# saminiir/level-ip

Measured on AMD Instinct MI355X. Metric: device-resident checksum GB/s over packet batch; % of HBM-read roofline, higher is better.
Workload: dtype u16

## Files before the change

### level-ip_amd/csrc/push_kernels.hip

```cpp
#include <hip/hip_runtime.h>

#include <stdint.h>

#include "seg_frame_dev.h"

namespace lvlip {

constexpr uint32_t PUSH_WAVES = 4;

__global__ __launch_bounds__(256) void k_push_count(lvlip_snd_flow* s, const lvlip_push_flow* w, uint32_t nflows,
                                                    lvlip_frame_desc* fd, uint8_t* sacked, lvlip_push_result* res) {
    const uint32_t lane = threadIdx.x & 63u;
    const uint64_t k64 = (uint64_t)blockIdx.x * PUSH_WAVES + (threadIdx.x >> 6);
    if (k64 >= nflows) return;
    const uint32_t k = (uint32_t)k64;
    const uint32_t una = s[k].snd_una, nxt = s[k].snd_nxt, seg0 = s[k].seg0, nseg = s[k].nseg;
    const lvlip_push_flow* t = w + k;
    const uint32_t q0 = t->q0, cap = t->cap;

    const uint32_t moved = seg0 != q0 ? nseg : 0u;
    if (seg0 > q0 && nseg <= cap) {
        for (uint64_t c0 = 0; c0 < nseg; c0 += 64u) {
            const uint64_t i = c0 + lane;
            uint4 d = make_uint4(0u, 0u, 0u, 0u);
            uint8_t b = 0;
            if (i < nseg) {
                d = load_global(reinterpret_cast<uint64_t>(fd + (seg0 + (uint32_t)i)));
                if (sacked) b = sacked[seg0 + (uint32_t)i];
            }
            __builtin_amdgcn_wave_barrier();
            if (i < nseg) {
                store_global(reinterpret_cast<uint64_t>(fd + (q0 + (uint32_t)i)), u32x4{d.x, d.y, d.z, d.w});
                if (sacked) sacked[q0 + (uint32_t)i] = b;
            }
        }
    }

    if (lane == 0u) {
        const uint32_t unsent = t->unsent, mss = t->mss, wnd = t->wnd;
        const uint32_t span = nxt - una;
        const uint32_t need = mss ? (uint32_t)(((uint64_t)unsent + mss - 1u) / mss) : 0u;
        uint32_t m = nseg < cap && (seg0 >= q0 || nseg == 0u) ? cap - nseg : 0u;
        m = min(m, min(t->push, need));
        const bool open = span <= wnd;
        const uint32_t room = open ? wnd - span : 0u;
        const uint32_t fit = open && unsent <= room ? need : (mss ? room / mss : 0u);
        m = min(m, fit);
        const uint64_t by = (uint64_t)m * mss;
        const uint32_t bytes = by < unsent ? (uint32_t)by : unsent;
        store_global(reinterpret_cast<uint64_t>(res + k), u32x4{m, bytes, q0 + nseg, moved});
        s[k].seg0 = q0;
    }
}

__global__ __launch_bounds__(256) void k_push(const lvlip_lro_flow* f, const lvlip_lro_result* lro,
                                              const lvlip_snd_flow* s, const lvlip_push_flow* w, uint32_t nflows,
                                              uint32_t nslots, const uint8_t* payload, uint8_t* base,
                                              lvlip_frame_desc* fd, uint8_t* sacked, lvlip_frame_desc* fd_out,
                                              const lvlip_push_result* res) {
    const uint32_t tl = threadIdx.x & (TSO_ROW - 1u);
    const uint64_t g64 = (uint64_t)blockIdx.x * TSO_SEGS + (threadIdx.x / TSO_ROW);
    const bool inside = g64 < nslots;
    const uint32_t g = inside ? (uint32_t)g64 : 0u;

    const uint32_t k = slot_owner<&lvlip_push_flow::slot0>(w, nflows, g);
    const lvlip_push_flow* t = w + k;
    const uint4 r = load_global(reinterpret_cast<uint64_t>(res + k));
    const uint32_t i = g - t->slot0;
    const bool live = inside && g >= t->slot0 && i < t->push && i < r.x;
    const uint32_t mss = t->mss, unsent = t->unsent;
    const uint64_t done = (uint64_t)i * mss;
    const uint32_t dlen = live ? (unsent - done < mss ? (uint32_t)(unsent - done) : mss) : 0u;
    const bool last = done + dlen == unsent;

    uint64_t slot = (uint64_t)t->slot_nxt + i;
    if (slot >= t->cap) slot -= t->cap;
    const uint64_t off = live ? t->ring_off + slot * t->stride : 0ull;
    const uint64_t F = reinterpret_cast<uint64_t>(base) + off;
    const uint64_t S = reinterpret_cast<uint64_t>(payload) + t->pay_off + done;
    uint32_t h[14];
    tso_frame(tl, live, h, F, S, dlen, last, [=](uint32_t(&hd)[14]) {
        const uint32_t* hw = reinterpret_cast<const uint32_t*>(t->hdr);
#pragma unroll
        for (int j = 0; j < 14; ++j) hd[j] = hw[j];
        hdr_put_ack(hd, __builtin_bswap32(f[k].rcv_nxt + (lro ? lro[k].delivered : 0u)));
        hd[12] = (hd[12] & 0xffff0000u) | bswap16u(s[k].win);
        return s[k].snd_nxt + (uint32_t)done;
    });

    if (inside && tl == 0u) {
        const u32x4 d = live ? u32x4{(uint32_t)off, (uint32_t)(off >> 32), (uint32_t)TSO_HDR + dlen, 0u}
                             : u32x4{0u, 0u, 0u, 0u};
        store_global(reinterpret_cast<uint64_t>(fd_out + g), d);
        if (live) {
            store_global(reinterpret_cast<uint64_t>(fd + (r.z + i)), d);
            if (sacked) sacked[r.z + i] = 0;
        }
    }
}

__global__ __launch_bounds__(256) void k_push_step(lvlip_snd_flow* s, lvlip_push_flow* w, uint32_t nflows,
                                                   const lvlip_push_result* res) {
    const uint32_t k = blockIdx.x * 256u + threadIdx.x;
    if (k >= nflows) return;
    uint2* sw = reinterpret_cast<uint2*>(s + k);
    uint2* ww = reinterpret_cast<uint2*>(w + k);
    const uint4 r = load_global(reinterpret_cast<uint64_t>(res + k));
    uint2 a = sw[0], q = sw[1], p = ww[0], u = ww[2], n = ww[4];
    const uint32_t cap = ww[3].x;
    a.y += r.y;
    q.y += r.x;
    const uint64_t pay = (((uint64_t)p.y << 32) | p.x) + r.y;
    p.x = (uint32_t)pay, p.y = (uint32_t)(pay >> 32);
    u.x -= r.y;
    const uint64_t nx = (uint64_t)n.x + r.x;
    n.x = (uint32_t)(nx >= cap ? nx - cap : nx);
    sw[0] = a, sw[1] = q;
    ww[0] = p, ww[2] = u, ww[4] = n;
}

}

extern "C" {

int lvlip_push_dev(const lvlip_lro_flow* f, const lvlip_lro_result* lro, lvlip_snd_flow* s, lvlip_push_flow* w,
                   uint32_t nflows, uint32_t nslots, const void* payload, void* base, lvlip_frame_desc* fd,
                   uint8_t* sacked, lvlip_frame_desc* fd_out, lvlip_push_result* res, void* stream) {
    if (nflows > LVLIP_LRO_MAX_FLOWS || nslots > LVLIP_MAX_BATCH) return LVLIP_EINVAL;
    if (nslots && (!payload || !base || !fd_out || nflows == 0)) return LVLIP_EINVAL;
    if (nflows == 0) return LVLIP_OK;
    if (!f || !s || !w || !fd || !res) return LVLIP_EINVAL;
    if (((uintptr_t)f & 7u) || ((uintptr_t)s & 7u) || ((uintptr_t)w & 7u) || ((uintptr_t)lro & 15u) ||
        ((uintptr_t)fd & 15u) || ((uintptr_t)fd_out & 15u) || ((uintptr_t)res & 15u))
        return LVLIP_EINVAL;
    hipStream_t st = (hipStream_t)stream;
    const uint32_t fgrid = (nflows + lvlip::PUSH_WAVES - 1u) / lvlip::PUSH_WAVES;
    hipLaunchKernelGGL(lvlip::k_push_count, dim3(fgrid), dim3(256), 0, st, s, w, nflows, fd, sacked, res);
    int rc = lvlip_launched("k_push_count");
    if (rc != LVLIP_OK) return rc;
    if (nslots) {
        const uint32_t grid = (uint32_t)(((uint64_t)nslots + lvlip::TSO_SEGS - 1u) / lvlip::TSO_SEGS);
        hipLaunchKernelGGL(lvlip::k_push, dim3(grid), dim3(256), 0, st, f, lro, s, w, nflows, nslots,
                           (const uint8_t*)payload, (uint8_t*)base, fd, sacked, fd_out, res);
        rc = lvlip_launched("k_push");
        if (rc != LVLIP_OK) return rc;
    }
    hipLaunchKernelGGL(lvlip::k_push_step, dim3((nflows + 255u) / 256u), dim3(256), 0, st, s, w, nflows, res);
    return lvlip_launched("k_push_step");
}

}
```

### level-ip_amd/csrc/seg_frame_dev.h

```cpp
#pragma once

#include <hip/hip_runtime.h>

#include <stdint.h>

#include "csum_dev.h"
#include "row_copy.h"
#include "tcp_hdr_dev.h"

namespace lvlip {

constexpr uint32_t TSO_ROW = 16;
constexpr uint32_t TSO_SEGS = 256 / TSO_ROW;
constexpr int TSO_U = 4;
constexpr int TSO_HDR = TCP_FRAME_HDR;

template <class PATCH>
__device__ __forceinline__ void tso_frame(uint32_t tl, bool live, uint32_t (&h)[14], uint64_t F, uint64_t S,
                                          uint32_t dlen, bool last, PATCH&& patch) {
    const int f = (int)(F & 15ull);
    const uint64_t D = F - (uint64_t)f;
    const int L = TSO_HDR + (int)dlen;
    const uint32_t nch = live ? (uint32_t)(f + L + 15) >> 4 : 0u;
    const uint32_t hk = (uint32_t)(f + TSO_HDR + 15) >> 4;
    const uint32_t sel = (F & 1ull) ? 0x02030001u : 0x03020100u;

    uint32_t acc = 0;
    uint4 keep = make_uint4(0u, 0u, 0u, 0u);
    for (uint32_t k0 = 0; k0 < nch; k0 += TSO_ROW * TSO_U) {
        uint4 v[TSO_U];
        row_gather<TSO_U, true>(S, f + TSO_HDR, dlen, nch, k0, tl, v);
#pragma unroll
        for (int u = 0; u < TSO_U; ++u) {
            const uint32_t k = k0 + (uint32_t)u * TSO_ROW + tl;
            acc = chunk_acc(v[u], sel, acc);
            if (k < nch) {
                if (k >= hk) store_chunk(D + 16ull * k, v[u], 0, min(16, f + L - (int)(16u * k)));
                else keep = v[u];
            }
        }
    }
    const uint32_t W = row_sum_dpp(acc);

    const uint32_t seq = patch(h);
    h[13] &= 0xffffu;
    h[4] = (h[4] & 0xffff0000u) | bswap16u(40u + dlen);
    h[6] &= 0xffff0000u;
    const uint32_t ipw = (h[3] >> 16) + halves(h[4]) + halves(h[5]) + halves(h[6]) + halves(h[7]) +
                         (h[8] & 0xffffu);
    h[6] |= (uint32_t)finish(0u, ipw);
    const uint32_t nseq = __builtin_bswap32(seq);
    h[9] = (h[9] & 0xffffu) | (nseq << 16);
    h[10] = (h[10] & 0xffff0000u) | (nseq >> 16);
    if (!last) h[11] &= ~(0x09u << 24);
    h[12] &= 0xffffu;
    const uint32_t thw = hdr_tcp_words(h);
    h[12] |= (uint32_t)finish(hdr_tcp_seed(h, 20u + dlen), thw + W) << 16;

    if (tl < hk && tl < nch) {
        const uint4 blk[4] = {make_uint4(h[0], h[1], h[2], h[3]), make_uint4(h[4], h[5], h[6], h[7]),
                              make_uint4(h[8], h[9], h[10], h[11]), make_uint4(h[12], h[13], 0u, 0u)};
        const uint4 hv = hdr_chunk(tl, f, blk);
        const uint4 v = make_uint4(keep.x | hv.x, keep.y | hv.y, keep.z | hv.z, keep.w | hv.w);
        store_chunk(D + 16ull * tl, v, tl == 0u ? f : 0, min(16, f + L - (int)(16u * tl)));
    }
}

}
```

### level-ip_amd/csrc/seg_kernels.hip

```cpp
#include <hip/hip_runtime.h>

#include <stdint.h>

#include "seg_frame_dev.h"

namespace lvlip {

__global__ __launch_bounds__(256) void k_tso(const uint8_t* payload, const lvlip_tso_send* s, uint32_t n,
                                             uint32_t nseg, uint8_t* out, lvlip_frame_desc* fd) {
    const uint32_t tl = threadIdx.x & (TSO_ROW - 1u);
    const uint64_t g64 = (uint64_t)blockIdx.x * TSO_SEGS + (threadIdx.x / TSO_ROW);
    bool live = g64 < nseg;
    const uint32_t g = live ? (uint32_t)g64 : 0u;

    const lvlip_tso_send* t = s + slot_owner<&lvlip_tso_send::seg0>(s, n, g);
    const uint32_t mss = t->mss, len = t->len;
    const uint32_t i = g - t->seg0;
    const uint64_t done = (uint64_t)i * mss;
    live = live && g >= t->seg0 && done < len;
    const uint32_t dlen = live ? (len - done < mss ? (uint32_t)(len - done) : mss) : 0u;
    const bool last = done + dlen == len;

    uint32_t h[14];
    {
        const uint32_t* hw = reinterpret_cast<const uint32_t*>(t->hdr);
#pragma unroll
        for (int k = 0; k < 14; ++k) h[k] = hw[k];
    }

    const uint64_t off = t->out_off + (uint64_t)i * t->stride;
    const uint64_t F = reinterpret_cast<uint64_t>(out) + off;
    const uint64_t S = reinterpret_cast<uint64_t>(payload) + t->payload_off + done;
    const uint32_t seq0 = __builtin_bswap32((h[9] >> 16) | (h[10] << 16));
    tso_frame(tl, live, h, F, S, dlen, last, [=](uint32_t(&)[14]) { return seq0 + (uint32_t)done; });
    if (fd && live && tl == 0u)
        store_global(reinterpret_cast<uint64_t>(fd + g), u32x4{(uint32_t)off, (uint32_t)(off >> 32), (uint32_t)TSO_HDR + dlen, 0u});
}

}

extern "C" {

int lvlip_tso_dev(const void* payload, const lvlip_tso_send* s, uint32_t n, uint32_t nseg, void* out,
                  lvlip_frame_desc* fd, void* stream) {
    if (n == 0) return LVLIP_OK;
    if (!payload || !s || !out || nseg == 0 || nseg > LVLIP_MAX_BATCH) return LVLIP_EINVAL;
    const uint32_t grid = (uint32_t)(((uint64_t)nseg + lvlip::TSO_SEGS - 1u) / lvlip::TSO_SEGS);
    hipLaunchKernelGGL(lvlip::k_tso, dim3(grid), dim3(256), 0, (hipStream_t)stream, (const uint8_t*)payload, s,
                       n, nseg, (uint8_t*)out, fd);
    return lvlip_launch_status(hipGetLastError(), "k_tso");
}

}
```

Before: 6883.

## Software-pipeline TSO payload loads and make k_tso a persistent grid-stride kernel

Measured after the change: 6882 (median of 2 runs). No clear change (-0.0%).

```diff
diff --git a/level-ip_amd/csrc/push_kernels.hip b/level-ip_amd/csrc/push_kernels.hip
--- a/level-ip_amd/csrc/push_kernels.hip
+++ b/level-ip_amd/csrc/push_kernels.hip
@@ -79,7 +79,7 @@
     const uint64_t F = reinterpret_cast<uint64_t>(base) + off;
     const uint64_t S = reinterpret_cast<uint64_t>(payload) + t->pay_off + done;
     uint32_t h[14];
-    tso_frame(tl, live, h, F, S, dlen, last, [=](uint32_t(&hd)[14]) {
+    tso_frame(tl, live, h, F, S, dlen, last, reinterpret_cast<uint64_t>(w), [=](uint32_t(&hd)[14]) {
         const uint32_t* hw = reinterpret_cast<const uint32_t*>(t->hdr);
 #pragma unroll
         for (int j = 0; j < 14; ++j) hd[j] = hw[j];
diff --git a/level-ip_amd/csrc/seg_frame_dev.h b/level-ip_amd/csrc/seg_frame_dev.h
--- a/level-ip_amd/csrc/seg_frame_dev.h
+++ b/level-ip_amd/csrc/seg_frame_dev.h
@@ -12,37 +12,79 @@
 
 constexpr uint32_t TSO_ROW = 16;
 constexpr uint32_t TSO_SEGS = 256 / TSO_ROW;
-constexpr int TSO_U = 4;
+constexpr int TSO_U = 3;
+constexpr uint32_t TSO_ROUND = TSO_ROW * TSO_U;
 constexpr int TSO_HDR = TCP_FRAME_HDR;
 
-template <class PATCH>
-__device__ __forceinline__ void tso_frame(uint32_t tl, bool live, uint32_t (&h)[14], uint64_t F, uint64_t S,
-                                          uint32_t dlen, bool last, PATCH&& patch) {
-    const int f = (int)(F & 15ull);
-    const uint64_t D = F - (uint64_t)f;
-    const int L = TSO_HDR + (int)dlen;
-    const uint32_t nch = live ? (uint32_t)(f + L + 15) >> 4 : 0u;
-    const uint32_t hk = (uint32_t)(f + TSO_HDR + 15) >> 4;
-    const uint32_t sel = (F & 1ull) ? 0x02030001u : 0x03020100u;
+struct tso_seg {
+    uint64_t D, A0;
+    uint32_t dlen;
+    uint32_t nch;
+    uint32_t sh;
+    uint32_t j0, j1;
+    int f;
+};
 
-    uint32_t acc = 0;
-    uint4 keep = make_uint4(0u, 0u, 0u, 0u);
-    for (uint32_t k0 = 0; k0 < nch; k0 += TSO_ROW * TSO_U) {
-        uint4 v[TSO_U];
-        row_gather<TSO_U, true>(S, f + TSO_HDR, dlen, nch, k0, tl, v);
+__device__ __forceinline__ tso_seg tso_seg_at(bool live, uint64_t F, uint64_t S, uint32_t dlen, uint64_t safe) {
+    tso_seg q;
+    q.f = (int)(F & 15ull);
+    q.D = F - (uint64_t)q.f;
+    const uint64_t A = S - (uint64_t)(q.f + TSO_HDR);
+    const bool has = live && dlen != 0u;
+    q.A0 = has ? A & ~15ull : safe;
+    q.sh = (uint32_t)(A & 15ull);
+    q.dlen = live ? dlen : 0u;
+    q.nch = live ? (uint32_t)(q.f + TSO_HDR + (int)dlen + 15) >> 4 : 0u;
+    q.j0 = has ? (uint32_t)(((S & ~15ull) - q.A0) >> 4) : 0u;
+    q.j1 = has ? (uint32_t)((((S + dlen - 1u) & ~15ull) - q.A0) >> 4) : 0u;
+    return q;
+}
+
+__device__ __forceinline__ void tso_issue(const tso_seg& q, uint32_t k0, uint32_t tl, uint4 (&x)[TSO_U + 1]) {
 #pragma unroll
-        for (int u = 0; u < TSO_U; ++u) {
-            const uint32_t k = k0 + (uint32_t)u * TSO_ROW + tl;
-            acc = chunk_acc(v[u], sel, acc);
-            if (k < nch) {
-                if (k >= hk) store_chunk(D + 16ull * k, v[u], 0, min(16, f + L - (int)(16u * k)));
-                else keep = v[u];
-            }
+    for (int u = 0; u < TSO_U; ++u) {
+        const uint32_t j = k0 + (uint32_t)u * TSO_ROW + tl;
+        x[u] = load_nt_global(q.A0 + 16ull * min(max(j, q.j0), q.j1));
+    }
+    x[TSO_U] = load_nt_global(q.A0 + 16ull * min(max(k0 + TSO_ROUND, q.j0), q.j1));
+}
+
+__device__ __forceinline__ uint32_t row_next(uint32_t v) {
+    return (uint32_t)__builtin_amdgcn_update_dpp(0, (int)v, 0x12F, 0xF, 0xF, false);
+}
+
+__device__ __forceinline__ void tso_consume(const tso_seg& q, uint32_t k0, uint32_t tl, const uint4 (&x)[TSO_U + 1],
+                                            uint32_t& acc, uint4& keep) {
+    const int lead = q.f + TSO_HDR;
+    const int L = TSO_HDR + (int)q.dlen;
+    const uint32_t hk = (uint32_t)(lead + 15) >> 4;
+    const uint32_t sel = (q.f & 1) ? 0x02030001u : 0x03020100u;
+#pragma unroll
+    for (int u = 0; u < TSO_U; ++u) {
+        const uint32_t k = k0 + (uint32_t)u * TSO_ROW + tl;
+        const int rel = (int)(16u * k) - lead;
+        const int jlo = min(max(-rel, 0), 16);
+        const int jhi = min(max((int)q.dlen - rel, 0), 16);
+        const uint4 own = x[u], nxt = x[u + 1];
+        const uint4 hi = make_uint4(row_next(tl == 0u ? nxt.x : own.x), row_next(tl == 0u ? nxt.y : own.y),
+                                    row_next(tl == 0u ? nxt.z : own.z), row_next(tl == 0u ? nxt.w : own.w));
+        const uint4 v = mask_chunk(funnel16(own, hi, q.sh), jlo, jhi);
+        acc = chunk_acc(v, sel, acc);
+        if (k < q.nch) {
+            if (k >= hk) store_chunk(q.D + 16ull * k, v, 0, min(16, q.f + L - (int)(16u * k)));
+            else keep = v;
         }
     }
+}
+
+__device__ __forceinline__ void tso_finish(const tso_seg& q, uint32_t tl, uint32_t (&h)[14], uint32_t acc,
+                                           const uint4 keep, bool last, uint32_t seq) {
+    const uint32_t dlen = q.dlen;
+    const int f = q.f;
+    const int L = TSO_HDR + (int)dlen;
+    const uint32_t hk = (uint32_t)(f + TSO_HDR + 15) >> 4;
     const uint32_t W = row_sum_dpp(acc);
 
-    const uint32_t seq = patch(h);
     h[13] &= 0xffffu;
     h[4] = (h[4] & 0xffff0000u) | bswap16u(40u + dlen);
     h[6] &= 0xffff0000u;
@@ -57,13 +99,33 @@
     const uint32_t thw = hdr_tcp_words(h);
     h[12] |= (uint32_t)finish(hdr_tcp_seed(h, 20u + dlen), thw + W) << 16;
 
-    if (tl < hk && tl < nch) {
+    if (tl < hk && tl < q.nch) {
         const uint4 blk[4] = {make_uint4(h[0], h[1], h[2], h[3]), make_uint4(h[4], h[5], h[6], h[7]),
                               make_uint4(h[8], h[9], h[10], h[11]), make_uint4(h[12], h[13], 0u, 0u)};
         const uint4 hv = hdr_chunk(tl, f, blk);
         const uint4 v = make_uint4(keep.x | hv.x, keep.y | hv.y, keep.z | hv.z, keep.w | hv.w);
-        store_chunk(D + 16ull * tl, v, tl == 0u ? f : 0, min(16, f + L - (int)(16u * tl)));
+        store_chunk(q.D + 16ull * tl, v, tl == 0u ? f : 0, min(16, f + L - (int)(16u * tl)));
     }
 }
 
+template <class PATCH>
+__device__ __forceinline__ void tso_frame(uint32_t tl, bool live, uint32_t (&h)[14], uint64_t F, uint64_t S,
+                                          uint32_t dlen, bool last, uint64_t safe, PATCH&& patch) {
+    const tso_seg q = tso_seg_at(live, F, S, dlen, safe);
+    uint32_t acc = 0;
+    uint4 keep = make_uint4(0u, 0u, 0u, 0u);
+    uint4 xa[TSO_U + 1], xb[TSO_U + 1];
+    tso_issue(q, 0u, tl, xa);
+    for (uint32_t k0 = 0;; k0 += 2u * TSO_ROUND) {
+        tso_issue(q, k0 + TSO_ROUND, tl, xb);
+        tso_consume(q, k0, tl, xa, acc, keep);
+        if (k0 + TSO_ROUND >= q.nch) break;
+        tso_issue(q, k0 + 2u * TSO_ROUND, tl, xa);
+        tso_consume(q, k0 + TSO_ROUND, tl, xb, acc, keep);
+        if (k0 + 2u * TSO_ROUND >= q.nch) break;
+    }
+    const uint32_t seq = patch(h);
+    tso_finish(q, tl, h, acc, keep, last, seq);
 }
+
+}
diff --git a/level-ip_amd/csrc/seg_kernels.hip b/level-ip_amd/csrc/seg_kernels.hip
--- a/level-ip_amd/csrc/seg_kernels.hip
+++ b/level-ip_amd/csrc/seg_kernels.hip
@@ -6,35 +6,102 @@
 
 namespace lvlip {
 
+constexpr int TSO_WAVES_PER_CU = 8;
+
+struct tso_cache {
+    uint32_t idx;
+    uint32_t seg0, len, mss, stride;
+    uint64_t out_off, pay_off;
+    uint32_t h[14];
+};
+
+struct tso_job {
+    tso_seg q;
+    uint64_t off;
+    uint32_t g;
+    uint32_t seq;
+    bool last;
+};
+
+__device__ __forceinline__ tso_job tso_resolve(uint64_t g64, uint32_t nseg, const lvlip_tso_send* s, uint32_t n,
+                                               tso_cache& c, const uint8_t* payload, uint8_t* out) {
+    bool live = g64 < nseg;
+    const uint32_t g = live ? (uint32_t)g64 : 0u;
+    if (live) {
+        const bool hit = c.idx < n && g >= c.seg0 && (uint64_t)(g - c.seg0) * c.mss < c.len;
+        if (!hit) {
+            c.idx = slot_owner<&lvlip_tso_send::seg0>(s, n, g);
+            const lvlip_tso_send* t = s + c.idx;
+            c.seg0 = t->seg0, c.len = t->len, c.mss = t->mss, c.stride = t->stride;
+            c.out_off = t->out_off, c.pay_off = t->payload_off;
+            const uint32_t* hw = reinterpret_cast<const uint32_t*>(t->hdr);
+#pragma unroll
+            for (int k = 0; k < 14; ++k) c.h[k] = hw[k];
+        }
+    }
+    const uint32_t i = g - c.seg0;
+    const uint64_t done = (uint64_t)i * c.mss;
+    live = live && g >= c.seg0 && done < c.len;
+    const uint32_t dlen = live ? (c.len - done < c.mss ? (uint32_t)(c.len - done) : c.mss) : 0u;
+    tso_job j;
+    j.g = g;
+    j.last = done + dlen == c.len;
+    j.off = c.out_off + (uint64_t)i * c.stride;
+    j.seq = __builtin_bswap32((c.h[9] >> 16) | (c.h[10] << 16)) + (uint32_t)done;
+    j.q = tso_seg_at(live, reinterpret_cast<uint64_t>(out) + j.off,
+                     reinterpret_cast<uint64_t>(payload) + c.pay_off + done, dlen, reinterpret_cast<uint64_t>(s));
+    return j;
+}
+
+__device__ __forceinline__ void tso_step(uint32_t tl, const uint4 (&xc)[TSO_U + 1], uint4 (&xi)[TSO_U + 1],
+                                         tso_job& cur, uint32_t& k0, uint64_t& g, uint64_t R, uint32_t (&hc)[14],
+                                         uint32_t& acc, uint4& keep, tso_cache& c, const uint8_t* payload,
+                                         const lvlip_tso_send* s, uint32_t n, uint32_t nseg, uint8_t* out,
+                                         lvlip_frame_desc* fd) {
+    const bool more = k0 + TSO_ROUND < cur.q.nch;
+    tso_job nx = cur;
+    uint32_t nk0 = k0 + TSO_ROUND;
+    if (!more) {
+        g += R;
+        nx = tso_resolve(g, nseg, s, n, c, payload, out);
+        nk0 = 0u;
+    }
+    tso_issue(nx.q, nk0, tl, xi);
+    tso_consume(cur.q, k0, tl, xc, acc, keep);
+    if (!more) {
+        tso_finish(cur.q, tl, hc, acc, keep, cur.last, cur.seq);
+        if (fd && tl == 0u)
+            store_global(reinterpret_cast<uint64_t>(fd + cur.g),
+                         u32x4{(uint32_t)cur.off, (uint32_t)(cur.off >> 32), (uint32_t)TSO_HDR + cur.q.dlen, 0u});
+        acc = 0u;
+#pragma unroll
+        for (int k = 0; k < 14; ++k) hc[k] = c.h[k];
+    }
+    cur = nx;
+    k0 = nk0;
+}
+
 __global__ __launch_bounds__(256) void k_tso(const uint8_t* payload, const lvlip_tso_send* s, uint32_t n,
                                              uint32_t nseg, uint8_t* out, lvlip_frame_desc* fd) {
     const uint32_t tl = threadIdx.x & (TSO_ROW - 1u);
-    const uint64_t g64 = (uint64_t)blockIdx.x * TSO_SEGS + (threadIdx.x / TSO_ROW);
-    bool live = g64 < nseg;
-    const uint32_t g = live ? (uint32_t)g64 : 0u;
+    const uint64_t R = (uint64_t)gridDim.x * TSO_SEGS;
+    uint64_t g = (uint64_t)blockIdx.x * TSO_SEGS + (threadIdx.x / TSO_ROW);
 
-    const lvlip_tso_send* t = s + slot_owner<&lvlip_tso_send::seg0>(s, n, g);
-    const uint32_t mss = t->mss, len = t->len;
-    const uint32_t i = g - t->seg0;
-    const uint64_t done = (uint64_t)i * mss;
-    live = live && g >= t->seg0 && done < len;
-    const uint32_t dlen = live ? (len - done < mss ? (uint32_t)(len - done) : mss) : 0u;
-    const bool last = done + dlen == len;
-
-    uint32_t h[14];
-    {
-        const uint32_t* hw = reinterpret_cast<const uint32_t*>(t->hdr);
+    tso_cache c = {};
+    c.idx = n;
+    tso_job cur = tso_resolve(g, nseg, s, n, c, payload, out);
+    uint32_t hc[14];
 #pragma unroll
-        for (int k = 0; k < 14; ++k) h[k] = hw[k];
+    for (int k = 0; k < 14; ++k) hc[k] = c.h[k];
+    uint32_t k0 = 0u, acc = 0u;
+    uint4 keep = make_uint4(0u, 0u, 0u, 0u);
+    uint4 xa[TSO_U + 1], xb[TSO_U + 1];
+    tso_issue(cur.q, 0u, tl, xa);
+    while (cur.q.nch != 0u) {
+        tso_step(tl, xa, xb, cur, k0, g, R, hc, acc, keep, c, payload, s, n, nseg, out, fd);
+        if (cur.q.nch == 0u) break;
+        tso_step(tl, xb, xa, cur, k0, g, R, hc, acc, keep, c, payload, s, n, nseg, out, fd);
     }
-
-    const uint64_t off = t->out_off + (uint64_t)i * t->stride;
-    const uint64_t F = reinterpret_cast<uint64_t>(out) + off;
-    const uint64_t S = reinterpret_cast<uint64_t>(payload) + t->payload_off + done;
-    const uint32_t seq0 = __builtin_bswap32((h[9] >> 16) | (h[10] << 16));
-    tso_frame(tl, live, h, F, S, dlen, last, [=](uint32_t(&)[14]) { return seq0 + (uint32_t)done; });
-    if (fd && live && tl == 0u)
-        store_global(reinterpret_cast<uint64_t>(fd + g), u32x4{(uint32_t)off, (uint32_t)(off >> 32), (uint32_t)TSO_HDR + dlen, 0u});
 }
 
 }
@@ -45,9 +112,12 @@
                   lvlip_frame_desc* fd, void* stream) {
     if (n == 0) return LVLIP_OK;
     if (!payload || !s || !out || nseg == 0 || nseg > LVLIP_MAX_BATCH) return LVLIP_EINVAL;
-    const uint32_t grid = (uint32_t)(((uint64_t)nseg + lvlip::TSO_SEGS - 1u) / lvlip::TSO_SEGS);
-    hipLaunchKernelGGL(lvlip::k_tso, dim3(grid), dim3(256), 0, (hipStream_t)stream, (const uint8_t*)payload, s,
-                       n, nseg, (uint8_t*)out, fd);
+    uint64_t grid = (uint64_t)lvlip_host::current_cus() * lvlip::TSO_WAVES_PER_CU / 4u;
+    const uint64_t need = ((uint64_t)nseg + lvlip::TSO_SEGS - 1u) / lvlip::TSO_SEGS;
+    if (grid > need) grid = need;
+    if (grid > 8u) grid &= ~7ull;
+    hipLaunchKernelGGL(lvlip::k_tso, dim3((uint32_t)grid), dim3(256), 0, (hipStream_t)stream,
+                       (const uint8_t*)payload, s, n, nseg, (uint8_t*)out, fd);
     return lvlip_launch_status(hipGetLastError(), "k_tso");
 }
 
```
